# ZhangXinWhut/SimWhisper-Codec

Measured on AMD Instinct MI355X. Metric: audio-sec/sec encode+decode (RTF^-1), 16kHz batch=32x10s, higher is better.
Workload: dtype split-f16 x3 encode (f32-class, f32 accumulate) / bf16 decode (f32 accumulate); 1 GPU; batch=32x10s @16kHz per GPU (32 utterances in all), encode()+decode(), 0.1*N(0,1) seed 1234, synthetic closed-form checkpoint (291M params); precision=mixed

## Files before the change

### simwhisper_codec_amd/_lib.py

```python
import ctypes as C
import os

import torch

HERE = os.path.dirname(os.path.abspath(__file__))
LIB_PATH = os.environ.get("SWC_LIB") or os.path.join(HERE, "libswc_hip.so")

F32, BF16, F16S, FP8 = 0, 1, 2, 3
F16S_ACT_SCALE = 64.0
FP8_ACT_SCALE = 16.0
ACT_NONE, ACT_GELU = 0, 1


class SwcError(RuntimeError):
    pass


class GemmArgs(C.Structure):
    _fields_ = [
        ("A", C.c_void_p), ("W", C.c_void_p), ("C", C.c_void_p),
        ("bias", C.c_void_p), ("gamma", C.c_void_p), ("residual", C.c_void_p),
        ("lda", C.c_int64), ("ldw", C.c_int64), ("ldc", C.c_int64), ("ldr", C.c_int64),
        ("M", C.c_int32), ("N", C.c_int32), ("K", C.c_int32),
        ("taps", C.c_int32), ("dil", C.c_int32), ("stride", C.c_int32), ("pad", C.c_int32),
# ... 182 lines not shown
    "swc_loudness_normalise": ([_P, _P, _P, _D, _D, _P, _L, _L, _P, _P, _I, _P], C.c_int),
}

ACTIVITY_MIN_FS, ACTIVITY_MAX_FS = 8000, 48000
ACTIVITY_MAX_N = 1 << 30
ACTIVITY_MAX_HANGOVER = 24000
ACTIVITY_SUBBLOCK, ACTIVITY_GROUP = 256, 64
ACTIVITY_TILE, ACTIVITY_THREADS = 4096, 256
ACTIVITY_THRESHOLDS, ACTIVITY_VALUES = 15, 8
ACTIVITY_UNMEASURED, ACTIVITY_PEAK_LIMITED = 1, 2
ACTIVITY_SIGNATURES = {
    "swc_activity_coefficients": ([_I, _D, C.POINTER(_D), C.POINTER(_I), C.POINTER(_I), C.POINTER(_D)], C.c_int),
    "swc_activity_workspace_bytes": ([_I, _L, _I], C.c_int64),
    "swc_activity": ([_P, _P, _L, _I, _D, _D, _P, _P, _P, _L, _P, _L, _I, _P], C.c_int),
    "swc_activity_normalise": ([_P, _P, _P, _D, _P, _L, _L, _P, _P, _I, _P], C.c_int),
}

TRACK_W, TRACK_P = 16, 32
TRACK_TABLE_ROWS, TRACK_TABLE_COLS = 35, 33
TRACK_MAX_RANGE = 1024
TRACK_MAX_N = 1 << 22
TRACK_MAX_SEGMENTS = 4096
TRACK_CHUNK, TRACK_LAG_BLOCK, TRACK_SPILL = 4096, 256, 256
TRACK_VALUES = 4
TRACK_DEFINED, TRACK_EDGE = 1, 2
FIT_VALUES, FIT_COUNTS = 4, 4
FIT_NO_DRIFT, FIT_NO_LAG, FIT_EDGE = 1, 2, 4
WARP_TAPS, WARP_PHASES, WARP_BLOCK, WARP_INFO = 32, 256, 256, 4
WARP_MAX_DRIFT = 0.01
WARP_MAX_LAG = 1 << 23
TRACK_SIGNATURES = {
    "swc_track_segments": ([_L, _I, _I], C.c_int64),
    "swc_lag_track_workspace_bytes": ([_I, _L, _L, _I, _I, _I], C.c_int64),
    "swc_lag_track": ([_P, _P, _P, _P, _L, _L, _P, _L, _I, _I, _I, _I, _P, _P, _P, _L, _P, _P, _L, _P, _L, _I, _P], C.c_int),
    "swc_lag_fit": ([_P, _P, _L, _P, _I, _P, _L, _D, _I, _P, _P, _I, _P], C.c_int),
    "swc_warp": ([_P, _P, _P, _L, _L, _P, _L, _P, _P, _L, _L, _P, _I, _P], C.c_int),
}

SEGMENTAL_MIN_WIN, SEGMENTAL_MAX_WIN = 64, 2048
SEGMENTAL_MAX_ORDER, SEGMENTAL_MAX_BANDS = 32, 64
SEGMENTAL_VALUES, SEGMENTAL_MEASURES = 8, 5
SEGMENTAL_SIGNATURES = {
    "swc_segmental_workspace_bytes": ([_I, _L, _I, _I, _I], C.c_int64),
    "swc_segmental": ([_P, _P, _P, _L, _I, _I, _I, _P, _P, _P, _P, _L, _P, _P, _L, _P, _L, _I, _P], C.c_int),
}

SUBDTW_MAX_PATCH = 256
SUBDTW_MAX_STEPS, SUBDTW_MAX_STRIDE = 4, 3
SUBDTW_MAX_FRAMES, SUBDTW_MAX_D = 8192, 32
SUBDTW_INFO = 4
SUBDTW_ST_OK, SUBDTW_ST_UNREACHABLE, SUBDTW_ST_UNDEFINED, SUBDTW_ST_QUERY = 0, 1, 2, 3
CMVN_BLOCK = 256
SUBDTW_SIGNATURES = {
    "swc_cmvn": ([_P, _P, _I, _I, _L, _P, _L, _I, _P], C.c_int),
    "swc_subdtw_workspace_bytes": ([_I, _I, _I, _I, _I], C.c_int64),
    "swc_subdtw": ([_P, _P, _P, _P, _I, _I, _I, _L, _I, _I, C.POINTER(C.c_int32), _I, _P, _P, _L, _P, _P, _P, _P, _L, _I, _P], C.c_int),
}

UNITS_MAX_GROUPS, UNITS_MAX_CODES = 8, 16384
UNITS_MAX_FRAMES = 8192
UNITS_CHUNK, UNITS_STRIP = 1024, 256
UNITS_USAGE_MAX_FRAMES = 1 << 24
UNITS_SIGNATURES = {
    "swc_code_usage": ([_P, _P, _P, _I, C.POINTER(C.c_int32), _I, _I, _P, _P, _P, _I, _P], C.c_int),
    "swc_code_compare": ([_P, _P, _P, _P, _P, _P, _I, C.POINTER(C.c_int32), _I, _I, _I, _P, _P, _P, _P, _P, _P, _P, _P, _P, _I, _P],
                         C.c_int),
}

ENTROPY_HEADER_BYTES = 24
ENTROPY_MAX_FRAMES, ENTROPY_MAX_GROUPS = 65536, 8
ENTROPY_MIN_LEVEL, ENTROPY_MAX_LEVEL, ENTROPY_MAX_CODES = 2, 16, 16384
ENTROPY_INC, ENTROPY_LIMIT, ENTROPY_MAX_RENORM = 24, 8192, 3
ENTROPY_E = {-1: "not a SWC2 image", -2: "unsupported version", -3: "groups, frames or levels outside the limits",
             -4: "truncated", -5: "inconsistent stream table", -6: "CRC mismatch"}
ENTROPY_SIGNATURES = {
    "swc_entropy_worst_bytes": ([_L, _I, C.POINTER(C.c_int32)], C.c_int64),
    "swc_entropy_workspace_bytes": ([C.POINTER(C.c_int64), _I, _I, C.POINTER(C.c_int32), C.POINTER(C.c_int64)], C.c_int64),
    "swc_entropy_encode_batch": ([_P, _P, _P, _I, C.POINTER(C.c_int32), _I, _I, _P, _L, _P, _P, _P, _P, _L, _I, _P], C.c_int),
    "swc_entropy_decode_batch": ([_P, _L, _P, _P, _P, _P, C.POINTER(C.c_int32), _I, _P, _L, _L, _L, _I, _I, _P, _P], C.c_int),
    "swc_entropy_parse": ([C.c_char_p, _L, _I, C.POINTER(C.c_int32), C.POINTER(C.c_int32), C.POINTER(C.c_int32), C.POINTER(C.c_int64),
                           C.POINTER(C.c_int64), C.POINTER(C.c_int32)], C.c_int),
}

_lib = None


def load():
    global _lib
    if _lib is not None:
        return _lib
    if not os.path.exists(LIB_PATH):
        raise SwcError(
            f"{LIB_PATH} is missing: build it with `python -m simwhisper_codec_amd.build` "
            "(there is no CPU or PyTorch fallback for the hot path)")
    lib = C.CDLL(LIB_PATH)
    for name, argtypes in SIGNATURES.items():
        fn = getattr(lib, name)
        fn.argtypes = argtypes
        fn.restype = C.c_int
    for table in (PLAIN, AUDIO_SIGNATURES, CODES_SIGNATURES, METRICS_SIGNATURES, QUALITY_SIGNATURES, FLAC_SIGNATURES,
                  FLAC_ENC_SIGNATURES, SPECTRAL_SIGNATURES, PITCH_SIGNATURES, ALIGN_SIGNATURES, MCD_SIGNATURES,
                  LOUDNESS_SIGNATURES, ACTIVITY_SIGNATURES, TRACK_SIGNATURES, SEGMENTAL_SIGNATURES, SUBDTW_SIGNATURES,
                  UNITS_SIGNATURES, ENTROPY_SIGNATURES):
        for name, (argtypes, restype) in table.items():
            fn = getattr(lib, name)
            fn.argtypes = argtypes
            fn.restype = restype
    _lib = lib
    return lib


def check(rc, what):
    if rc != 0:
        msg = load().swc_last_error().decode("utf-8", "replace")
        raise SwcError(f"{what} failed (rc={rc}): {msg}")


def exported_symbols():
    return list(SIGNATURES) + list(PLAIN)
```

### simwhisper_codec_amd/build.py

```python
import os
import shutil
import subprocess
import sys

HERE = os.path.dirname(os.path.abspath(__file__))
ROOT = os.path.dirname(HERE)
CSRC = os.path.join(HERE, "csrc")
LIB_PATH = os.path.join(HERE, "libswc_hip.so")
SOURCES = ["swc_api.hip", "swc_gemm.hip", "swc_gemm_skinny.hip", "swc_attention.hip", "swc_attention16.hip", "swc_pointwise.hip", "swc_convnext.hip", "swc_mlp.hip", "swc_convnext64.hip", "swc_projln.hip",
           "swc_resample.hip", "swc_codes.hip", "swc_stoi.hip", "swc_flac_gpu.hip", "swc_flac_enc.hip", "swc_spectral.hip", "swc_pitch.hip", "swc_align.hip", "swc_mcd.hip", "swc_loudness.hip", "swc_activity.hip", "swc_track.hip", "swc_segmental.hip", "swc_subdtw.hip", "swc_units.hip", "swc_entropy.hip"]
ARCH = "gfx950"
_MAX_ILP = ["-mllvm", "-amdgpu-sched-strategy=max-ilp"]
EXTRA_FLAGS = {"swc_attention16.hip": ["-fno-slp-vectorize"], "swc_convnext.hip": ["-fno-slp-vectorize"] + _MAX_ILP,
               "swc_mlp.hip": ["-fno-slp-vectorize"] + _MAX_ILP, "swc_convnext64.hip": ["-fno-slp-vectorize"] + _MAX_ILP,
               "swc_projln.hip": ["-fno-slp-vectorize"] + _MAX_ILP,
               "swc_gemm.hip": _MAX_ILP,
               "swc_track.hip": ["-ffp-contract=off"],
               "swc_segmental.hip": ["-ffp-contract=off"],
               "swc_subdtw.hip": ["-ffp-contract=off"]}


def _hipcc():
    for cand in (os.environ.get("HIPCC"), "/opt/rocm/bin/hipcc", shutil.which("hipcc")):
        if cand and os.path.exists(cand):
            return cand
    raise RuntimeError("hipcc not found (set HIPCC or install ROCm under /opt/rocm)")


def _stale():
    if not os.path.exists(LIB_PATH):
        return True
    t = os.path.getmtime(LIB_PATH)
    deps = [os.path.join(CSRC, f) for f in os.listdir(CSRC) if f.endswith((".hip", ".h"))] + [os.path.join(ROOT, "include", h) for h in ("swc.h", "swc_audio.h", "swc_codes.h", "swc_metrics.h", "swc_quality.h", "swc_flac.h", "swc_flac_enc.h", "swc_spectral.h", "swc_pitch.h", "swc_align.h", "swc_mcd.h", "swc_loudness.h", "swc_activity.h", "swc_track.h", "swc_segmental.h", "swc_subdtw.h", "swc_units.h", "swc_entropy.h")]
    return any(os.path.getmtime(d) > t for d in deps)


def build_library(force=False, verbose=False):
    if not force and not _stale():
        return LIB_PATH
    hipcc = _hipcc()
    objdir = os.path.join(HERE, "build")
    os.makedirs(objdir, exist_ok=True)
    common = [
        hipcc, f"--offload-arch={ARCH}", "-O3", "-std=c++17", "-fPIC",
        "-ffp-contract=on",
        "-I", os.path.join(ROOT, "include"), "-I", CSRC,
    ]
    objs = []
    procs = []
    for src in SOURCES:
        obj = os.path.join(objdir, src.replace(".hip", ".o"))
        cmd = common + EXTRA_FLAGS.get(src, []) + ["-c", os.path.join(CSRC, src), "-o", obj]
        if verbose:
            cmd.insert(1, "-Rpass-analysis=kernel-resource-usage")
        procs.append((src, subprocess.Popen(cmd, stdout=subprocess.PIPE, stderr=subprocess.STDOUT, text=True)))
        objs.append(obj)
    for src, p in procs:
        out, _ = p.communicate()
        if p.returncode != 0:
            raise RuntimeError(f"hipcc failed on {src}:\n{out}")
        if verbose:
            print(out)
    tmp = LIB_PATH + ".tmp"
    link = [hipcc, f"--offload-arch={ARCH}", "-shared", "-fPIC", "-o", tmp] + objs
    r = subprocess.run(link, stdout=subprocess.PIPE, stderr=subprocess.STDOUT, text=True)
    if r.returncode != 0:
        raise RuntimeError(f"link failed:\n{r.stdout}")
    os.replace(tmp, LIB_PATH)
    stamp_commit()
    return LIB_PATH


IO_LIB_PATH = os.path.join(HERE, "libswc_io.so")
IO_SOURCES = ["swc_flac.c"]


def build_io_library(force=False):
    srcs = [os.path.join(CSRC, f) for f in IO_SOURCES]
    deps = srcs + [os.path.join(ROOT, "include", "swc_flac.h")]
    if not force and os.path.exists(IO_LIB_PATH) and all(os.path.getmtime(f) <= os.path.getmtime(IO_LIB_PATH) for f in deps):
        return IO_LIB_PATH
    cc = next((c for c in (os.environ.get("CC"), shutil.which("gcc"), shutil.which("cc"), shutil.which("clang")) if c), None)
    if cc is None:
        raise RuntimeError("no C compiler found for libswc_io.so (set CC)")
    tmp = IO_LIB_PATH + ".tmp"
    r = subprocess.run([cc, "-O2", "-std=c99", "-Wall", "-I", os.path.join(ROOT, "include"), "-shared", "-fPIC", "-o", tmp] + srcs,
                       stdout=subprocess.PIPE, stderr=subprocess.STDOUT, text=True)
    if r.returncode != 0:
        raise RuntimeError(f"building libswc_io.so failed:\n{r.stdout}")
    os.replace(tmp, IO_LIB_PATH)
    return IO_LIB_PATH


FLAC_CHECK_PATH = os.path.join(HERE, "swc_flac_check")
FLAC_CHECK_SOURCES = ["swc_flac_check.cpp", "swc_flac.c"]


def build_flac_check(force=False, sanitize=True):
    srcs = [os.path.join(CSRC, f) for f in FLAC_CHECK_SOURCES]
    deps = srcs + [os.path.join(CSRC, "swc_flac_frame.h"), os.path.join(ROOT, "include", "swc_flac.h")]
    target = FLAC_CHECK_PATH if sanitize else FLAC_CHECK_PATH + "_plain"
    if not force and os.path.exists(target) and all(os.path.getmtime(f) <= os.path.getmtime(target) for f in deps):
        return target
    cxx = next((c for c in (os.environ.get("CXX"), shutil.which("g++"), shutil.which("clang++")) if c), None)
    cc = next((c for c in (os.environ.get("CC"), shutil.which("gcc"), shutil.which("cc"), shutil.which("clang")) if c), None)
    if cxx is None or cc is None:
        raise RuntimeError("no C / C++ compiler found for swc_flac_check (set CC / CXX)")
    san = ["-fsanitize=address,undefined", "-fno-sanitize-recover=all", "-fno-omit-frame-pointer", "-g", "-O1"] if sanitize else ["-O2"]
    tag = "san" if sanitize else "plain"
    inc = ["-I", os.path.join(ROOT, "include"), "-I", CSRC]
    objdir = os.path.join(HERE, "build")
    os.makedirs(objdir, exist_ok=True)
    obj_c, obj_x = os.path.join(objdir, f"flac_check_io_{tag}.o"), os.path.join(objdir, f"flac_check_main_{tag}.o")
    tmp = target + ".tmp"
    static = ["-static-libasan", "-static-libubsan"] if sanitize else []
    steps = [[cc, "-std=c99", "-Wall"] + san + inc + ["-c", srcs[1], "-o", obj_c],
# ... 96 lines not shown
```

### simwhisper_codec_amd/codec.py

```python
import contextlib
import functools
import logging
import math
import os
import threading

import torch
import torch.nn as nn
import yaml

from . import bitstream, metrics, ops, packed, spec, trace
from ._lib import SwcError

PRECISIONS = {"fp32": ("f32", "f32"), "mixed": ("f16s", "bf16"), "mixed_f32": ("f32", "bf16"), "bf16": ("bf16", "bf16"),
              "fp8": ("bf16", "bf16"), "fp8_fc1": ("bf16", "bf16"), "f16s": ("f16s", "f16s")}
_TORCH_DT = {"f32": torch.float32, "bf16": torch.bfloat16, "f16s": torch.float16}


_TLS = threading.local()


def _on_model_device(fn):
    @functools.wraps(fn)
    def wrapped(self, *a, **k):
# ... 639 lines not shown

    def _cast(self, x, dt, K=None):
        if dt == torch.bfloat16 and x.dtype != dt:
            return ops.cast_bf16(x)
        if dt == torch.float16 and x.dtype != dt:
            return ops.cast_f16s(x, x.shape[-1] if K is None else K)
        return x

    @staticmethod
    def _mm(A, pw, M, N, K, out_dtype=None, **kw):
        if out_dtype == torch.float16:
            kw["out_scale"] = ops.F16S_ACT_SCALE
        elif out_dtype == ops.FP8_T:
            kw["out_scale"] = ops.FP8_ACT_SCALE
        return ops.gemm(A, pw.w, M, N, K, alpha=pw.alpha, out_dtype=out_dtype, **kw)

    def _transformer(self, h, lens, B, T, layers, H, dt, row_start=None):
        D = h.shape[-1]
        M = h.shape[0]
        fp8 = dt == ops.FP8_T
        adt = torch.bfloat16 if fp8 else dt
        lnB, lnT = (B, T) if row_start is None else (1, M)
        fused = self._mlp_fused(layers, M, dt)
        x = None
        for i, L in enumerate(layers):
            if x is None:
                x = ops.layernorm(h, L.ln1[0], L.ln1[1], 1e-5, B=lnB, t_in=lnT, C_=D, out_dtype=dt)
            qkv = self._mm(x, L.wqkv, M, 3 * D, D, lda=D, bias=L.bqkv, out_dtype=adt)
            a = ops.attention(qkv, lens, B, T, H, row_start=row_start, rows=M)
            if fp8:
                a = ops.cast_fp8(a)
            F_ = L.b1.shape[0]
            nxt = layers[i + 1].ln1 if i + 1 < len(layers) else None
            if fused and self.layer_fusion >= 2 and getattr(L, "wts", None) is not None:
                _, x = ops.layer_tail(a, h, L.wts, L.bo, L.ln2[0], L.ln2[1], 1e-5, L.b1, L.b2, M=M, D=D, F=F_, next_ln=nxt,
                                      fc1_dtype=L.w1.w.dtype, fc1_alpha=L.w1.alpha,
                                      operands=torch.float16 if getattr(L, "t16", False) else torch.bfloat16)
                continue
            self._mm(a, L.wo, M, D, D, lda=D, bias=L.bo, residual=h, out=h)
            if fused and self.layer_fusion == 1:
                _, x = ops.mlp_block(h, L.ln2[0], L.ln2[1], 1e-5, L.ws, L.b1, L.b2, M=M, D=D, F=F_, next_ln=nxt)
                continue
            dt1 = L.w1.w.dtype if L.w1.w.dtype == ops.FP8_T else dt
            x = ops.layernorm(h, L.ln2[0], L.ln2[1], 1e-5, B=lnB, t_in=lnT, C_=D, out_dtype=dt1)
            f = self._mm(x, L.w1, M, F_, D, lda=D, bias=L.b1, act=ops.ACT_GELU, out_dtype=dt)
            self._mm(f, L.w2, M, D, F_, lda=F_, bias=L.b2, residual=h, out=h)
            x = None
        return h

    fused_layer_mlp_min_rows = 64 * 160
    layer_fusion = 2

    def _mlp_fused(self, layers, M, dt):
        if dt != torch.bfloat16 or M < self.fused_layer_mlp_min_rows or self.layer_fusion <= 0:
            return False
        if any(getattr(L, "wts" if self.layer_fusion >= 2 else "ws", None) is None for L in layers):
            return False
        if self.fused_layer_mlp_min_rows <= 0:
            return True
        tiles = spec.cdiv(M, 64)
        rounds = spec.cdiv(tiles, self.CUS)
        return tiles >= 0.6 * rounds * self.CUS

    convnext_f16 = False

    @staticmethod
    def _cx_f16_safe(sd, p, n_blocks, C):
        lim = 65504.0 / 8
        for i in range(n_blocks):
            b_ = f"{p}convnext.{i}."
            w1, w2 = sd[b_ + "pwconv1.weight"], sd[b_ + "pwconv2.weight"]
            if not (bool(torch.isfinite(w1).all()) and bool(torch.isfinite(w2).all())):
                return False
            if float(w1.abs().max()) >= lim or float(w2.abs().max()) >= lim:
                return False
            if math.sqrt(C) * float(sd[b_ + "norm.weight"].abs().max()) + float(sd[b_ + "norm.bias"].abs().max()) >= lim:
                return False
        return True

    layer_tail_f16 = True
    vocos_head_split_f16 = True
    decoder_io_split_f16 = False
    upsample_split_f16 = False
    conv1_split_f16 = True
    varlen_packing = True
    PACK_BELOW = 0.9

    def _pack_plan(self, lens_host, T, dt, dev):
        B = len(lens_host)
        total = sum(lens_host)
        if (not self.varlen_packing or dt == torch.float32 or total == 0 or total >= self.PACK_BELOW * B * T):
            return None, B * T
        cu, acc = [], 0
        for v in lens_host:
            cu.append(acc)
            acc += v
        return self._dev_ints(cu, dev), total

    def _res_units(self, h, units, B, T, C, dt):
        M = B * T
        for u in units:
            y = ops.snake_aa(h, u["a0"], u["b0"], u["f0"], B=B, T=T, C_=C, out_dtype=dt)
            y = self._mm(y, u["w1"], M, C, C, lda=C, ldw=7 * C, bias=u["c1"], taps=7, dil=u["dil"], pad=3 * u["dil"],
                         t_in=T, t_out=T)
            y = ops.snake_aa(y, u["a2"], u["b2"], u["f2"], B=B, T=T, C_=C, out_dtype=dt)
            self._mm(y, u["w3"], M, C, C, lda=C, bias=u["c3"], residual=h, out=h)
        return h

    def _logmel(self, wav, n_dev, n_host, P):
        with trace.stage("mel"):
            return self._logmel_impl(wav, n_dev, n_host, P)

    def _logmel_impl(self, wav, n_dev, n_host, P):
        B = wav.shape[0]
        Tm = min(spec.MEL_FRAMES, max(spec.mel_len(n) for n in n_host) + 2)
        fr = ops.mel_frames(wav, n_dev, spec.CHUNK_SAMPLES, B=B, T=Tm)
        M = B * Tm
        dft = self._mm(fr, P.dft, M, 402, 400, lda=400)
        pw = ops.mel_power(dft, 402, M, 208)
        mp = self._mm(pw, P.melw, M, P.n_mel, 208, lda=208)
        umax = torch.full((B,), -10.0 if Tm < spec.MEL_FRAMES else float("-inf"), device=wav.device, dtype=torch.float32)
        ops.mel_logmax(mp, P.n_mel, umax, B=B, T=Tm, n_mel=P.n_mel)
        mel = ops.mel_final(mp, P.n_mel, umax, B=B, T=Tm, n_mel=P.n_mel, ldo=P.c1k, out_dtype=P.c1dt)
        return mel, Tm

    def _encoder(self, mel, Tm, t_full, tok_host, P):
        with trace.stage("encoder"):
            return self._encoder_impl(mel, Tm, t_full, tok_host, P)

    def _encoder_impl(self, mel, Tm, t_full, tok_host, P):
        B, dt, D = mel.shape[0], P.edt, P.D
        dev = mel.device
        Ttok = max(1, min(t_full, max(tok_host)))
        K1 = P.c1k
        if K1 != P.n_mel:
            if mel.shape[-1] != K1:
                mel = torch.nn.functional.pad(mel.to(torch.float32), (0, K1 - mel.shape[-1]))
            mel = ops.cast_f16s(mel.view(B * Tm, K1), K1)
        c1 = self._mm(mel, P.c1w, B * Tm, D, K1, lda=K1, ldw=3 * K1, bias=P.c1b, taps=3, pad=1, t_in=Tm,
                      t_out=Tm, out_dtype=dt)
        h = self._mm(c1, P.c2w, B * Ttok, D, D, lda=D, ldw=3 * D, bias=P.c2b, taps=3, stride=2, pad=1, t_in=Tm, t_out=Ttok)
        tok_c = [min(t, Ttok) for t in tok_host]
        lens = self._dev_ints(tok_c, dev)
        row_start, total = self._pack_plan(tok_c, Ttok, P.enc_ldt, dev)
        if row_start is not None:
            h = ops.pack_rows(h, row_start, lens, B=B, T=Ttok, total=total)
        self._transformer(h, lens, B, Ttok, P.enc_layers, P.He, P.enc_ldt, row_start=row_start)
        s = P.stack
        tds_full = spec.cdiv(t_full, s)
        Tds = min(tds_full, spec.cdiv(Ttok, s) + 64)
        hn = ops.layernorm(h, P.enc_ln[0], P.enc_ln[1], 1e-5, B=B, t_in=Ttok, t_out=Tds * s, C_=D, lens=lens, out_dtype=dt,
                           row_start=row_start)
        return hn, Tds

    def _downsample(self, hn, B, Tds, P):
        with trace.stage("downsample"):
            return self._downsample_impl(hn, B, Tds, P)

    def _downsample_impl(self, hn, B, Tds, P):
        dt, s, D = P.edt, P.stack, P.D
        hd = self._mm(hn, P.inw, B * Tds, P.hid, s * D, lda=s * D, bias=P.inb)
        self._res_units(hd, P.down_units, B, Tds, P.hid, dt)
        z = self._mm(self._cast(hd, dt), P.tlw, B * Tds, P.lat, P.hid, lda=P.hid, bias=P.tlb)
        return z.view(B, Tds, P.lat)

    def _encode_mel(self, mel, Tm, t_full, tok_host, P):
        hn, Tds = self._encoder(mel, Tm, t_full, tok_host, P)
        z = self._downsample(hn, mel.shape[0], Tds, P)
        return z, Tds, [spec.cdiv(t, P.stack) for t in tok_host]

    VOCOS_HALO_FRAMES = 80

    def _upsample(self, zq, B, T, P):
        with trace.stage("upsample"):
            return self._upsample_impl(zq, B, T, P)

    def _upsample_impl(self, zq, B, T, P):
        dt, s, D = getattr(P, "udt", P.ddt), P.stack, P.Dd
        h = self._mm(self._cast(zq, dt), P.flw, B * T, P.uhid, P.lat, lda=P.lat, bias=P.flb)
        self._res_units(h, P.up_units, B, T, P.uhid, dt)
        x = self._mm(self._cast(h, dt), P.tsw, B * T, s * D, P.uhid, lda=P.uhid, bias=P.tsb)
        return x.view(B * s * T, D)

    def _decoder(self, x, lat_host, B, Tt, P):
        with trace.stage("decoder"):
            return self._decoder_impl(x, lat_host, B, Tt, P)

    def _decoder_impl(self, x, lat_host, B, Tt, P):
        dt, dev, D = P.ddt, x.device, P.Dd
        lens_h = [min(l * P.stack, Tt) for l in lat_host]
        lens = self._dev_ints(lens_h, dev)
        row_start, total = self._pack_plan(lens_h, Tt, dt, dev)
        if row_start is not None:
            x = ops.pack_rows(x, row_start, lens, B=B, T=Tt, total=total)
        self._transformer(x, lens, B, Tt, P.dec_layers, P.Hd, dt, row_start=row_start)
        io16 = getattr(P, "io16", dt == torch.float16)
        hn = ops.layernorm(x, P.dec_ln[0], P.dec_ln[1], 1e-5, B=B, t_in=Tt, C_=D, lens=lens,
                           out_dtype=torch.float16 if io16 else dt, row_start=row_start)
        y3 = self._mm(hn.view(B * Tt, -1), P.d1w, B * Tt, 3 * D, D, lda=D)
        Tv = 2 * Tt
        if io16:
            d1 = ops.deconv_col2im(y3, P.d1b, B=B, T=Tt, C_=D, s=2, t_out=Tv + 1, out_dtype=torch.float32)
# ... 566 lines not shown
```

### simwhisper_codec_amd/ops.py

```python
import ctypes as C
import math

import torch

from . import _lib
from ._lib import ACT_GELU, ACT_NONE, BF16, F16S, F16S_ACT_SCALE, F32, FP8, FP8_ACT_SCALE

FP8_T = torch.float8_e4m3fn
_DT = {torch.float32: F32, torch.bfloat16: BF16, torch.float16: F16S, FP8_T: FP8}


def _w(dtype, cols):
    return 2 * cols if dtype == torch.float16 else cols

PROFILER = None
LEGACY_ATTENTION = False


def _stream():
    return C.c_void_p(torch._C._cuda_getCurrentRawStream(torch._C._cuda_getDevice()))


def _ptr(t):
    return C.c_void_p(t.data_ptr()) if t is not None else C.c_void_p(0)
# ... 225 lines not shown
    return out


def layernorm(x, w, b, eps, *, B, t_in, C_, t_out=None, lens=None, out=None, out_dtype=torch.float32, row_start=None):
    lib = _lib.load()
    _chk(x, "layernorm x", torch.float32)
    t_out = t_in if t_out is None else t_out
    if out is None:
        out = torch.empty((B, t_out, _w(out_dtype, C_)), device=x.device, dtype=out_dtype)
    _lib.check(lib.swc_layernorm(_ptr(x), _ptr(out), _ptr(w), _ptr(b), _ptr(lens), B, t_in, t_out, C_, eps,
                                 _DT[out.dtype], _ptr(row_start), _stream()), "swc_layernorm")
    return out


def pack_rows(x, row_start, lens, *, B, T, total):
    lib = _lib.load()
    _chk(x, "pack_rows x"); _chk(row_start, "pack_rows row_start", torch.int32); _chk(lens, "pack_rows lens", torch.int32)
    Cw = x.shape[-1]
    out = torch.empty((total, Cw), device=x.device, dtype=x.dtype)
    _lib.check(lib.swc_pack_rows(_ptr(x), _ptr(out), _ptr(row_start), _ptr(lens), B, T, Cw * x.element_size(), _stream()),
               "swc_pack_rows")
    return out


def dwconv7_ln(x, w7, bias, ln_w, ln_b, eps, *, B, T, C_, out=None, out_dtype=torch.float32):
    lib = _lib.load()
    _chk(x, "dwconv7_ln x", torch.float32)
    if out is None:
        out = torch.empty((B, T, C_), device=x.device, dtype=out_dtype)
    _lib.check(lib.swc_dwconv7_ln(_ptr(x), _ptr(out), _ptr(w7), _ptr(bias), _ptr(ln_w), _ptr(ln_b), B, T, C_, eps,
                                  _DT[out.dtype], _stream()), "swc_dwconv7_ln")
    return out


def snake_aa(x, alpha, beta, filt12, *, B, T, C_, out=None, out_dtype=torch.float32):
    lib = _lib.load()
    _chk(x, "snake_aa x", torch.float32)
    if out is None:
        out = torch.empty((B, T, _w(out_dtype, C_)), device=x.device, dtype=out_dtype)
    f = (C.c_float * 12)(*[float(v) for v in filt12])
    _lib.check(lib.swc_snake_aa(_ptr(x), _ptr(out), _ptr(alpha), _ptr(beta), f, B, T, C_, _DT[out.dtype],
                                _stream()), "swc_snake_aa")
    return out


FSQ_LEVELS = (8, 7, 6, 6)


def fsq_encode(z, ldz, lens, consts12, *, B, T, t_pad, G, levels=FSQ_LEVELS):
    lib = _lib.load()
    _chk(z, "fsq_encode z", torch.float32); _chk(lens, "fsq_encode lens", torch.int32)
    zq = torch.empty((B, t_pad, 4 * G), device=z.device, dtype=torch.float32)
    codes = torch.empty((G, B, t_pad), device=z.device, dtype=torch.int32)
    k = (C.c_float * 12)(*[float(v) for v in consts12])
    lv = (C.c_int32 * 4)(*[int(v) for v in levels])
    _lib.check(lib.swc_fsq_encode_levels(_ptr(z), ldz, _ptr(zq), _ptr(codes), _ptr(lens), k, lv, B, T, t_pad, G, _stream()),
               "swc_fsq_encode_levels")
    return zq, codes


def fsq_decode(codes, lens, *, B, T, G, ldq=None, levels=FSQ_LEVELS):
    lib = _lib.load()
    _chk(codes, "fsq_decode codes", torch.int64); _chk(lens, "fsq_decode lens", torch.int32)
    ldq = 4 * G if ldq is None else ldq
    zq = torch.empty((B, T, ldq), device=codes.device, dtype=torch.float32)
    lv = (C.c_int32 * 4)(*[int(v) for v in levels])
    _lib.check(lib.swc_fsq_decode_levels(_ptr(codes), _ptr(zq), ldq, _ptr(lens), lv, B, T, G, _stream()), "swc_fsq_decode_levels")
    return zq


def mel_frames(wav, n, n_pad, *, B, T):
    lib = _lib.load()
    _chk(wav, "mel_frames wav", torch.float32); _chk(n, "mel_frames n", torch.int32)
    frames = torch.empty((B, T, 400), device=wav.device, dtype=torch.float32)
    _lib.check(lib.swc_mel_frames(_ptr(wav), wav.stride(0), _ptr(n), n_pad, _ptr(frames), B, T, _stream()),
               "swc_mel_frames")
    return frames


def mel_power(dft, ld, rows, ldp):
    lib = _lib.load()
    pw = torch.empty((rows, ldp), device=dft.device, dtype=torch.float32)
    _lib.check(lib.swc_mel_power(_ptr(dft), ld, _ptr(pw), ldp, rows, _stream()), "swc_mel_power")
    return pw


def mel_logmax(mel, ld, umax, *, B, T, n_mel):
    lib = _lib.load()
    _lib.check(lib.swc_mel_logmax(_ptr(mel), ld, _ptr(umax), B, T, n_mel, _stream()), "swc_mel_logmax")


def mel_final(mel, ld, umax, *, B, T, n_mel, ldo, out_dtype=torch.float32):
    lib = _lib.load()
    out = torch.empty((B, T, ldo), device=mel.device, dtype=out_dtype)
    _lib.check(lib.swc_mel_final(_ptr(mel), ld, _ptr(umax), _ptr(out), ldo, B, T, n_mel, _DT[out_dtype], _stream()),
               "swc_mel_final")
    return out


def deconv_col2im(y3, bias, *, B, T, C_, s, t_out, ldo=None, out_dtype=torch.float32):
    lib = _lib.load()
    ldo = C_ if ldo is None else ldo
    out = torch.empty((B, t_out, ldo), device=y3.device, dtype=out_dtype)
    _lib.check(lib.swc_deconv_col2im(_ptr(y3), _ptr(bias), _ptr(out), ldo, B, T, C_, s, t_out, _DT[out_dtype],
                                     _stream()), "swc_deconv_col2im")
    return out


def istft_spec(h, ldh, rows, lds, out_dtype=torch.float32):
    lib = _lib.load()
    s = torch.empty((rows, _w(out_dtype, lds)), device=h.device, dtype=out_dtype)
    _lib.check(lib.swc_istft_spec(_ptr(h), ldh, _ptr(s), lds, rows, _DT[out_dtype], _stream()), "swc_istft_spec")
    return s


def istft_ola(frames, window_sq, *, B, T):
    lib = _lib.load()
    wav = torch.empty((B, T * 160), device=frames.device, dtype=torch.float32)
    _lib.check(lib.swc_istft_ola(_ptr(frames), _ptr(window_sq), _ptr(wav), B, T, _stream()), "swc_istft_ola")
    return wav


def cast_bf16(x):
    lib = _lib.load()
    _chk(x, "cast_bf16 x", torch.float32)
    x = x.contiguous()
    y = torch.empty(x.shape, device=x.device, dtype=torch.bfloat16)
    _lib.check(lib.swc_cast_f32_bf16(_ptr(x), _ptr(y), x.numel(), _stream()), "swc_cast_f32_bf16")
    return y


def cast_fp8(x, scale=FP8_ACT_SCALE):
    lib = _lib.load()
    _chk(x, "cast_fp8 x")
    if x.dtype not in (torch.float32, torch.bfloat16):
        raise _lib.SwcError(f"cast_fp8: expected f32 or bf16, got {x.dtype}")
    x = x.contiguous()
    y = torch.empty(x.shape, device=x.device, dtype=FP8_T)
    _lib.check(lib.swc_cast_fp8(_ptr(x), _DT[x.dtype], _ptr(y), x.numel(), scale, _stream()), "swc_cast_fp8")
    return y


def cast_f16s(x, K, scale=F16S_ACT_SCALE, ldx=None):
    lib = _lib.load()
    _chk(x, "cast_f16s x", torch.float32)
    rows = x.numel() // x.shape[-1]
    ldx = x.stride(-2) if ldx is None else ldx
    y = torch.empty((rows, 2 * K), device=x.device, dtype=torch.float16)
    _lib.check(lib.swc_cast_f32_f16s(_ptr(x), ldx, _ptr(y), rows, K, scale, _stream()), "swc_cast_f32_f16s")
    return y


def gather_rows(ptrs_dev, nbytes_dev, n_rows, ld_elems, dtype, device):
    lib = _lib.load()
    out = torch.empty((n_rows, ld_elems), device=device, dtype=dtype)
    _lib.check(lib.swc_gather_rows(_ptr(ptrs_dev), _ptr(nbytes_dev), _ptr(out), ld_elems * out.element_size(), n_rows,
                                   _stream()), "swc_gather_rows")
    return out


def pcm16_to_f32(pcm):
    lib = _lib.load()
    _chk(pcm, "pcm16_to_f32 pcm", torch.int16)
    if not pcm.is_contiguous():
        raise _lib.SwcError("pcm16_to_f32: contiguous input expected")
    out = torch.empty(pcm.shape, device=pcm.device, dtype=torch.float32)
# ... 1157 lines not shown
```

Baseline: 15680 audio-s/s.

## Fuse mel framing, DFT GEMM and power spectrum into one MFMA kernel

Adds a single kernel that builds reflect-padded windowed frames directly from the waveform, multiplies them against an interleaved real/imag DFT basis with fp32 MFMA, and writes the power spectrum. The frames tensor and the 402-column DFT output no longer round-trip through global memory, and two launches go away. The basis is repacked once and cached per weight pointer. The new kernel hand-rolls LDS-DMA double buffering and swizzling, so its numerics and throughput depend on matching the old GEMM path. The mel stage is a small share of the full encode+decode work.

```diff
diff --git a/include/swc_spectral_ends.h b/include/swc_spectral_ends.h
--- /dev/null
+++ b/include/swc_spectral_ends.h
@@ -0,0 +1,17 @@
+#ifndef SWC_SPECTRAL_ENDS_H_
+#define SWC_SPECTRAL_ENDS_H_
+
+#include <stdint.h>
+
+#ifdef __cplusplus
+extern "C" {
+#endif
+
+int swc_mel_dft_power(const float* wav, int64_t ld_wav, const int32_t* n, int32_t n_pad, const float* dft_ri,
+                      float* pw, int64_t ldp, int32_t B, int32_t T, void* stream);
+
+#ifdef __cplusplus
+}
+#endif
+
+#endif
diff --git a/simwhisper_codec_amd/_lib.py b/simwhisper_codec_amd/_lib.py
--- a/simwhisper_codec_amd/_lib.py
+++ b/simwhisper_codec_amd/_lib.py
@@ -288,6 +288,10 @@
                            C.POINTER(C.c_int64), C.POINTER(C.c_int32)], C.c_int),
 }
 
+SPECTRAL_ENDS_SIGNATURES = {
+    "swc_mel_dft_power": ([_P, _L, _P, _I, _P, _P, _L, _I, _I, _P], C.c_int),
+}
+
 _lib = None
 
 
@@ -307,7 +311,7 @@
     for table in (PLAIN, AUDIO_SIGNATURES, CODES_SIGNATURES, METRICS_SIGNATURES, QUALITY_SIGNATURES, FLAC_SIGNATURES,
                   FLAC_ENC_SIGNATURES, SPECTRAL_SIGNATURES, PITCH_SIGNATURES, ALIGN_SIGNATURES, MCD_SIGNATURES,
                   LOUDNESS_SIGNATURES, ACTIVITY_SIGNATURES, TRACK_SIGNATURES, SEGMENTAL_SIGNATURES, SUBDTW_SIGNATURES,
-                  UNITS_SIGNATURES, ENTROPY_SIGNATURES):
+                  UNITS_SIGNATURES, ENTROPY_SIGNATURES, SPECTRAL_ENDS_SIGNATURES):
         for name, (argtypes, restype) in table.items():
             fn = getattr(lib, name)
             fn.argtypes = argtypes
diff --git a/simwhisper_codec_amd/build.py b/simwhisper_codec_amd/build.py
--- a/simwhisper_codec_amd/build.py
+++ b/simwhisper_codec_amd/build.py
@@ -8,7 +8,7 @@
 CSRC = os.path.join(HERE, "csrc")
 LIB_PATH = os.path.join(HERE, "libswc_hip.so")
 SOURCES = ["swc_api.hip", "swc_gemm.hip", "swc_gemm_skinny.hip", "swc_attention.hip", "swc_attention16.hip", "swc_pointwise.hip", "swc_convnext.hip", "swc_mlp.hip", "swc_convnext64.hip", "swc_projln.hip",
-           "swc_resample.hip", "swc_codes.hip", "swc_stoi.hip", "swc_flac_gpu.hip", "swc_flac_enc.hip", "swc_spectral.hip", "swc_pitch.hip", "swc_align.hip", "swc_mcd.hip", "swc_loudness.hip", "swc_activity.hip", "swc_track.hip", "swc_segmental.hip", "swc_subdtw.hip", "swc_units.hip", "swc_entropy.hip"]
+           "swc_resample.hip", "swc_codes.hip", "swc_stoi.hip", "swc_flac_gpu.hip", "swc_flac_enc.hip", "swc_spectral.hip", "swc_pitch.hip", "swc_align.hip", "swc_mcd.hip", "swc_loudness.hip", "swc_activity.hip", "swc_track.hip", "swc_segmental.hip", "swc_subdtw.hip", "swc_units.hip", "swc_entropy.hip", "swc_spectral_ends.hip"]
 ARCH = "gfx950"
 _MAX_ILP = ["-mllvm", "-amdgpu-sched-strategy=max-ilp"]
 EXTRA_FLAGS = {"swc_attention16.hip": ["-fno-slp-vectorize"], "swc_convnext.hip": ["-fno-slp-vectorize"] + _MAX_ILP,
@@ -31,7 +31,7 @@
     if not os.path.exists(LIB_PATH):
         return True
     t = os.path.getmtime(LIB_PATH)
-    deps = [os.path.join(CSRC, f) for f in os.listdir(CSRC) if f.endswith((".hip", ".h"))] + [os.path.join(ROOT, "include", h) for h in ("swc.h", "swc_audio.h", "swc_codes.h", "swc_metrics.h", "swc_quality.h", "swc_flac.h", "swc_flac_enc.h", "swc_spectral.h", "swc_pitch.h", "swc_align.h", "swc_mcd.h", "swc_loudness.h", "swc_activity.h", "swc_track.h", "swc_segmental.h", "swc_subdtw.h", "swc_units.h", "swc_entropy.h")]
+    deps = [os.path.join(CSRC, f) for f in os.listdir(CSRC) if f.endswith((".hip", ".h"))] + [os.path.join(ROOT, "include", h) for h in ("swc.h", "swc_audio.h", "swc_codes.h", "swc_metrics.h", "swc_quality.h", "swc_flac.h", "swc_flac_enc.h", "swc_spectral.h", "swc_pitch.h", "swc_align.h", "swc_mcd.h", "swc_loudness.h", "swc_activity.h", "swc_track.h", "swc_segmental.h", "swc_subdtw.h", "swc_units.h", "swc_entropy.h", "swc_spectral_ends.h")]
     return any(os.path.getmtime(d) > t for d in deps)
 
 
diff --git a/simwhisper_codec_amd/codec.py b/simwhisper_codec_amd/codec.py
--- a/simwhisper_codec_amd/codec.py
+++ b/simwhisper_codec_amd/codec.py
@@ -745,6 +745,7 @@
     vocos_head_split_f16 = True
     decoder_io_split_f16 = False
     upsample_split_f16 = False
+    spectral_fusion = True
     conv1_split_f16 = True
     varlen_packing = True
     PACK_BELOW = 0.9
@@ -770,6 +771,16 @@
             self._mm(y, u["w3"], M, C, C, lda=C, bias=u["c3"], residual=h, out=h)
         return h
 
+    def _dft_ri(self, P):
+        key = (P.dft.w.data_ptr(), P.dft.w.device)
+        st = self.__dict__.get("_dft_ri_cache")
+        if st is None or st[0] != key:
+            ri = ops.mel_dft_pack(P.dft.w)
+            if not torch.cuda.is_current_stream_capturing():
+                torch.cuda.current_stream().synchronize()
+            st = self.__dict__["_dft_ri_cache"] = (key, ri)
+        return st[1]
+
     def _logmel(self, wav, n_dev, n_host, P):
         with trace.stage("mel"):
             return self._logmel_impl(wav, n_dev, n_host, P)
@@ -777,10 +788,13 @@
     def _logmel_impl(self, wav, n_dev, n_host, P):
         B = wav.shape[0]
         Tm = min(spec.MEL_FRAMES, max(spec.mel_len(n) for n in n_host) + 2)
-        fr = ops.mel_frames(wav, n_dev, spec.CHUNK_SAMPLES, B=B, T=Tm)
         M = B * Tm
-        dft = self._mm(fr, P.dft, M, 402, 400, lda=400)
-        pw = ops.mel_power(dft, 402, M, 208)
+        if self.spectral_fusion:
+            pw = ops.mel_dft_power(wav, n_dev, spec.CHUNK_SAMPLES, self._dft_ri(P), B=B, T=Tm)
+        else:
+            fr = ops.mel_frames(wav, n_dev, spec.CHUNK_SAMPLES, B=B, T=Tm)
+            dft = self._mm(fr, P.dft, M, 402, 400, lda=400)
+            pw = ops.mel_power(dft, 402, M, 208)
         mp = self._mm(pw, P.melw, M, P.n_mel, 208, lda=208)
         umax = torch.full((B,), -10.0 if Tm < spec.MEL_FRAMES else float("-inf"), device=wav.device, dtype=torch.float32)
         ops.mel_logmax(mp, P.n_mel, umax, B=B, T=Tm, n_mel=P.n_mel)
diff --git a/simwhisper_codec_amd/csrc/swc_spectral_ends.hip b/simwhisper_codec_amd/csrc/swc_spectral_ends.hip
--- /dev/null
+++ b/simwhisper_codec_amd/csrc/swc_spectral_ends.hip
@@ -0,0 +1,181 @@
+#include "swc_mfma.h"
+#include "swc_spectral_ends.h"
+
+namespace {
+
+constexpr int SE_BM = 128;
+constexpr int SE_NP = 416;
+constexpr int SE_K = 400;
+constexpr int SE_BINS = 208;
+constexpr int SE_WM = 4, SE_WN = 2;
+constexpr int SE_MT = 2, SE_NT = 13;
+constexpr int SE_NTHREADS = SE_WM * SE_WN * 64;
+constexpr int SE_A_BYTES = SE_BM * 128;
+constexpr int SE_W_BYTES = SE_NP * 128;
+constexpr int SE_A_BASE = 2 * SE_W_BYTES;
+constexpr int SE_LDS = 2 * (SE_W_BYTES + SE_A_BYTES);
+static_assert(2 * SE_W_BYTES <= 128 * 1024, "LDS-DMA destinations stay below 128 KiB");
+constexpr int SE_NKT = (SE_K + 31) / 32;
+constexpr int SE_WSWEEPS = SE_NP / 8;
+static_assert(SE_BM * SE_BINS * 4 <= SE_LDS, "the output tile must fit the stage buffers");
+static_assert(SE_WM * SE_MT * 16 == SE_BM && SE_WN * SE_NT * 16 == SE_NP, "wave layout");
+
+__device__ __forceinline__ int se_swz(int row) { return ((row >> 1) ^ ((row >> 4) << 1)) & 7; }
+__device__ __forceinline__ int se_off(int row, int chunk) { return row * 128 + ((chunk ^ se_swz(row)) << 4); }
+
+__global__ __launch_bounds__(SE_NTHREADS) void mel_dft_power_kernel(const float* __restrict__ wav, long ld_wav,
+                                                                       const int* __restrict__ n, int n_pad,
+                                                                       const float* __restrict__ W, float* __restrict__ pw,
+                                                                       long ldp, int T, int M, int vec_ok) {
+    extern __shared__ __attribute__((aligned(16))) char smem[];
+    const int tid = threadIdx.x;
+    const int lane = tid & 63;
+    const int wave = __builtin_amdgcn_readfirstlane(tid >> 6);
+    const int wr = wave / SE_WN, wc = wave % SE_WN;
+    const int bm = blockIdx.x * SE_BM;
+    const unsigned smem_base = __builtin_amdgcn_readfirstlane(lds_addr_of(smem));
+
+    const int a_c = tid & 7;
+    const float* a_wb[2];
+    int a_s0[2], a_nb[2], a_lds[2];
+#pragma unroll
+    for (int i = 0; i < 2; ++i) {
+        const int row = (tid >> 3) + 64 * i;
+        const int r = bm + row;
+        const bool ok = r < M;
+        const int b = ok ? r / T : 0;
+        const int t = ok ? r - b * T : 0;
+        a_nb[i] = ok ? n[b] : 0;
+        a_wb[i] = wav + (long)b * ld_wav;
+        a_s0[i] = t * 160 - 200 + 4 * a_c;
+        a_lds[i] = SE_A_BASE + se_off(row, a_c);
+    }
+    auto a_load = [&](int i, int kt) -> float4 {
+        const int s0 = a_s0[i] + 32 * kt;
+        const int nb = a_nb[i];
+        const float* wb = a_wb[i];
+        if (vec_ok && s0 >= 0 && s0 + 3 < nb && s0 + 3 < n_pad) return *reinterpret_cast<const float4*>(wb + s0);
+        float e[4];
+#pragma unroll
+        for (int q = 0; q < 4; ++q) {
+            int s = s0 + q;
+            if (s < 0) s = -s;
+            if (s >= n_pad) s = 2 * (n_pad - 1) - s;
+            e[q] = s < nb ? wb[s] : 0.f;
+        }
+        return make_float4(e[0], e[1], e[2], e[3]);
+    };
+    const bool a_tail_ok = a_c < 4;
+
+    const char* w_bytes = reinterpret_cast<const char*>(W);
+    auto w_stage = [&](int kt, int stage) {
+        const unsigned sb = smem_base + stage * SE_W_BYTES;
+        for (int q = wave; q < SE_WSWEEPS; q += SE_WM * SE_WN) {
+            const int row = 8 * q + (lane >> 3);
+            int chunk = (lane & 7) ^ se_swz(row);
+            if (kt == SE_NKT - 1) chunk &= 3;
+            glds16(w_bytes + (long)row * (SE_K * 4) + (kt * 8 + chunk) * 16, sb + q * 1024);
+        }
+    };
+    auto fence = [&]() {
+        asm volatile("s_waitcnt vmcnt(0)" ::: "memory");
+        __syncthreads();
+    };
+
+    f32x4 acc[SE_MT][SE_NT];
+#pragma unroll
+    for (int i = 0; i < SE_MT; ++i)
+#pragma unroll
+        for (int j = 0; j < SE_NT; ++j) acc[i][j] = (f32x4){0.f, 0.f, 0.f, 0.f};
+
+    const int fr = lane & 15, fh = lane >> 4;
+    const int a_row0 = wr * (SE_MT * 16) + fr;
+    const int b_row0 = wc * (SE_NT * 16) + fr;
+
+    w_stage(0, 0);
+#pragma unroll
+    for (int i = 0; i < 2; ++i) *reinterpret_cast<float4*>(smem + a_lds[i]) = a_load(i, 0);
+    fence();
+
+    for (int kt = 0; kt < SE_NKT; ++kt) {
+        const int cur = kt & 1;
+        const bool more = kt + 1 < SE_NKT;
+        const bool a_next = more && (kt + 1 < SE_NKT - 1 || a_tail_ok);
+        float4 an[2];
+        if (more) w_stage(kt + 1, cur ^ 1);
+        if (a_next) {
+#pragma unroll
+            for (int i = 0; i < 2; ++i) an[i] = a_load(i, kt + 1);
+        }
+        const char* sa = smem + SE_A_BASE + cur * SE_A_BYTES;
+        const char* sb = smem + cur * SE_W_BYTES;
+        const int ng = kt == SE_NKT - 1 ? 1 : 2;
+        for (int g = 0; g < ng; ++g) {
+            uint4 fa[SE_MT], fb[SE_NT];
+#pragma unroll
+            for (int j = 0; j < SE_NT; ++j) fb[j] = *reinterpret_cast<const uint4*>(sb + se_off(b_row0 + 16 * j, fh + 4 * g));
+#pragma unroll
+            for (int i = 0; i < SE_MT; ++i) fa[i] = *reinterpret_cast<const uint4*>(sa + se_off(a_row0 + 16 * i, fh + 4 * g));
+#pragma unroll
+            for (int e = 0; e < 4; ++e)
+#pragma unroll
+                for (int i = 0; i < SE_MT; ++i) {
+                    const float av = __uint_as_float(reinterpret_cast<const unsigned*>(&fa[i])[e]);
+#pragma unroll
+                    for (int j = 0; j < SE_NT; ++j) {
+                        const float bv = __uint_as_float(reinterpret_cast<const unsigned*>(&fb[j])[e]);
+                        acc[i][j] = __builtin_amdgcn_mfma_f32_16x16x4f32(bv, av, acc[i][j], 0, 0, 0);
+                    }
+                }
+        }
+        if (a_next) {
+#pragma unroll
+            for (int i = 0; i < 2; ++i) *reinterpret_cast<float4*>(smem + (cur ^ 1) * SE_A_BYTES + a_lds[i]) = an[i];
+        }
+        fence();
+    }
+
+    float* so = reinterpret_cast<float*>(smem);
+#pragma unroll
+    for (int i = 0; i < SE_MT; ++i) {
+        const int row = wr * (SE_MT * 16) + 16 * i + fr;
+#pragma unroll
+        for (int j = 0; j < SE_NT; ++j) {
+            const int bin = wc * (SE_NT * 8) + 8 * j + 2 * fh;
+            float v[2];
+#pragma unroll
+            for (int h = 0; h < 2; ++h) {
+                const float re = acc[i][j][2 * h], im = acc[i][j][2 * h + 1];
+                const float m = sqrtf(__fadd_rn(__fmul_rn(re, re), __fmul_rn(im, im)));
+                v[h] = bin + h < 201 ? __fmul_rn(m, m) : 0.f;
+            }
+            *reinterpret_cast<float2*>(so + row * SE_BINS + bin) = make_float2(v[0], v[1]);
+        }
+    }
+    __syncthreads();
+    const int rows = min(SE_BM, M - bm);
+    for (int q = tid; q < rows * (SE_BINS / 4); q += SE_NTHREADS) {
+        const int row = q / (SE_BINS / 4), c4 = q - row * (SE_BINS / 4);
+        *reinterpret_cast<float4*>(pw + (long)(bm + row) * ldp + 4 * c4) = *reinterpret_cast<const float4*>(so + row * SE_BINS + 4 * c4);
+    }
+}
+
+}
+
+extern "C" int swc_mel_dft_power(const float* wav, int64_t ld_wav, const int32_t* n, int32_t n_pad, const float* dft_ri,
+                                 float* pw, int64_t ldp, int32_t B, int32_t T, void* stream) {
+    SWC_CHECK_ARG(wav && n && dft_ri && pw, "swc_mel_dft_power: null pointer");
+    SWC_CHECK_ARG(n_pad >= 400 && B <= 65535, "swc_mel_dft_power: bad n_pad/B");
+    SWC_CHECK_ARG((long)(T - 1) * 160 + 199 < 2L * n_pad - 1, "swc_mel_dft_power: T too large for n_pad");
+    if (B <= 0 || T <= 0) return SWC_OK;
+    SWC_CHECK_ARG((long)B * T < (1L << 31) - SE_BM, "swc_mel_dft_power: too many rows");
+    SWC_CHECK_ARG(ldp >= SE_BINS && ldp % 4 == 0 && aligned16(pw), "swc_mel_dft_power: pw rows not 16-byte aligned or ldp < 208");
+    SWC_CHECK_ARG(aligned16(dft_ri), "swc_mel_dft_power: basis not 16-byte aligned");
+    const int vec_ok = aligned16(wav) && ld_wav % 4 == 0;
+    const int M = B * T;
+    SWC_ENABLE_LDS(mel_dft_power_kernel, SE_LDS, "swc_mel_dft_power");
+    hipLaunchKernelGGL(mel_dft_power_kernel, dim3((unsigned)((M + SE_BM - 1) / SE_BM)), dim3(SE_NTHREADS), SE_LDS,
+                       (hipStream_t)stream, wav, (long)ld_wav, n, n_pad, dft_ri, pw, (long)ldp, T, M, vec_ok);
+    SWC_CHECK_LAUNCH("swc_mel_dft_power");
+    return SWC_OK;
+}
diff --git a/simwhisper_codec_amd/ops.py b/simwhisper_codec_amd/ops.py
--- a/simwhisper_codec_amd/ops.py
+++ b/simwhisper_codec_amd/ops.py
@@ -331,6 +331,32 @@
     lib = _lib.load()
     pw = torch.empty((rows, ldp), device=dft.device, dtype=torch.float32)
     _lib.check(lib.swc_mel_power(_ptr(dft), ld, _ptr(pw), ldp, rows, _stream()), "swc_mel_power")
+    return pw
+
+
+def mel_dft_pack(dft):
+    _chk(dft, "mel_dft_pack dft", torch.float32)
+    if tuple(dft.shape) != (402, 400):
+        raise _lib.SwcError(f"mel_dft_pack: the basis is [402][400], got {tuple(dft.shape)}")
+    out = torch.zeros((416, 400), device=dft.device, dtype=torch.float32)
+    out[0:402:2] = dft[:201]
+    out[1:402:2] = dft[201:]
+    return out
+
+
+def mel_dft_power(wav, n, n_pad, dft_ri, *, B, T, ldp=208, out=None):
+    lib = _lib.load()
+    _chk(wav, "mel_dft_power wav", torch.float32); _chk(n, "mel_dft_power n", torch.int32)
+    _chk(dft_ri, "mel_dft_power dft_ri", torch.float32)
+    if tuple(dft_ri.shape) != (416, 400) or not dft_ri.is_contiguous():
+        raise _lib.SwcError("mel_dft_power: dft_ri is the contiguous [416][400] operand of mel_dft_pack")
+    if wav.dim() != 2 or wav.shape[0] < B or wav.stride(1) != 1 or n.numel() < B:
+        raise _lib.SwcError("mel_dft_power: wav is [B][>= max n] with unit column stride, n holds B lengths")
+    pw = torch.empty((max(B * T, 0), ldp), device=wav.device, dtype=torch.float32) if out is None else out
+    if B <= 0 or T <= 0:
+        return pw
+    _lib.check(lib.swc_mel_dft_power(_ptr(wav), wav.stride(0), _ptr(n), n_pad, _ptr(dft_ri), _ptr(pw), ldp, B, T, _stream()),
+               "swc_mel_dft_power")
     return pw
 
 
```

Result: no change. 15740 audio-s/s, median of 6 (+0.4%).
